# matsengrp/linearham

Hardware: AMD Instinct MI355X
Metric: phylo-HMM log-likelihood evals/sec (100-leaf x 400-site family) (higher is better)
Workload: dtype f64

## Files before the change

### include/linearham_amd.h

```cpp
#ifndef LINEARHAM_AMD_H_
#define LINEARHAM_AMD_H_

#include <stddef.h>
#include <stdint.h>

#ifdef __cplusplus
extern "C" {
#endif

#define LH_ABI_VERSION 1

typedef struct lh_family lh_family;

typedef struct {
  int32_t n_genes;
  const int32_t* offsets;
  const int32_t* xmsa_inds;
} lh_segments;

typedef struct {
  int32_t n_rows;
  int32_t n_left;
  int32_t n_right;
  const double* enter_trans;
// ... 31 lines not shown
} lh_family_desc;

typedef struct {
  double* rates;
  double* xmsa_emission;
  double* forward;
  int32_t* scaler_counts;
} lh_eval_outputs;

const char* lh_last_error(void);
int lh_device_count(void);

int lh_warmup(void);
int lh_set_device(int32_t device);
void* lh_host_alloc(size_t bytes);
void lh_host_free(void* p);

int lh_family_create(const lh_family_desc* desc, lh_family** out);
void lh_family_destroy(lh_family* fam);

int64_t lh_forward_size(const lh_family* fam);
int64_t lh_scaler_size(const lh_family* fam);

int lh_family_info(const lh_family* fam, int32_t* n_patterns, int32_t* n_unique_columns);

int lh_family_consensus_sets(const lh_family* fam);

const char* lh_family_prune_form(const lh_family* fam);

const char* lh_family_forward_form(const lh_family* fam);

int lh_family_forward_dj_samples(const lh_family* fam);

int lh_family_set_extended_range(lh_family* fam, int enable);

typedef struct {
  int32_t n_rows, n_left, n_right, n_states;
  const int32_t* left_rows;
  const int32_t* left_dense;
  const double* left_lo;
  const double* left_trans;
  const double* enter_lo;
  const int32_t* right_dense;
  const int32_t* right_first;
  const double* gene_prob;
  const double* nti_landing_in;
  const double* nti_transition;
  const double* nti_landing_out;
  const double* landing_in;
  const double* right_trans;
  const double* exit_nlo;
  const double* exit_trans;
  const double* exit_li;
  const double* prod;
} lh_sampler_junction;

typedef struct {
  lh_sampler_junction vd, dj;
} lh_sampler_desc;

int lh_family_set_sampler(lh_family* fam, const lh_sampler_desc* desc);

int32_t lh_sample_words(const lh_family* fam);
int32_t lh_sample_states(const lh_family* fam);

int lh_eval_sample_batch(lh_family* fam, int32_t n, int32_t n_tips, int32_t max_depth, const int32_t* ops,
// ... 317 lines not shown
```

### linearham_amd/capi.py

```python
import ctypes as C
import os

import numpy as np

_HERE = os.path.dirname(os.path.abspath(__file__))

c_i32p = C.POINTER(C.c_int32)
c_u8p = C.POINTER(C.c_uint8)
c_f64p = C.POINTER(C.c_double)


class _Segments(C.Structure):
    _fields_ = [("n_genes", C.c_int32), ("offsets", c_i32p), ("xmsa_inds", c_i32p)]


class _Junction(C.Structure):
    _fields_ = [("n_rows", C.c_int32), ("n_left", C.c_int32), ("n_right", C.c_int32),
                ("enter_trans", c_f64p), ("enter_lo", c_f64p), ("left_trans", c_f64p),
                ("left_lo", c_f64p), ("left_xmsa", c_i32p), ("right_gp_nli", c_f64p),
                ("right_ntt", c_f64p), ("right_nlo", c_f64p), ("right_trans", c_f64p),
                ("right_gp_li", c_f64p), ("right_xmsa", c_i32p), ("nti_xmsa", c_i32p),
                ("exit_nlo", c_f64p), ("exit_trans", c_f64p), ("exit_gp_li", c_f64p)]


class _FamilyDesc(C.Structure):
    _fields_ = [("abi_version", C.c_int32), ("has_d", C.c_int32), ("n_seqs", C.c_int32),
                ("n_sites", C.c_int32), ("msa", c_u8p), ("n_xmsa", C.c_int32),
                ("xmsa_site", c_i32p), ("xmsa_naive_base", c_u8p),
                ("vpadding", _Segments), ("vgerm", _Segments), ("dgerm", _Segments),
                ("jgerm", _Segments), ("jpadding", _Segments),
                ("vgerm_gene_prob", c_f64p), ("vpadding_transition", c_f64p),
                ("vgerm_trans_prod", c_f64p), ("jpadding_transition", c_f64p),
                ("vd", _Junction), ("dj", _Junction)]


class _EvalOutputs(C.Structure):
    _fields_ = [("rates", c_f64p), ("xmsa_emission", c_f64p), ("forward", c_f64p),
                ("scaler_counts", c_i32p)]


EXPORTS = ["lh_last_error", "lh_device_count", "lh_family_create", "lh_family_destroy",
           "lh_forward_size", "lh_scaler_size", "lh_family_info", "lh_family_consensus_sets", "lh_schedule_tree", "lh_eval_batch",
           "lh_eval_batch_device", "lh_forward_batch", "lh_asr_batch", "lh_asr_batch_device",
           "lh_profile_enable", "lh_profile_read", "lh_asr_profile_read", "lh_family_set_extended_range", "lh_warmup", "lh_host_alloc", "lh_host_free", "lh_family_set_sampler",
           "lh_sample_words", "lh_sample_states", "lh_eval_sample_batch", "lh_set_device", "lh_family_status",
           "lh_eval_sample_batch_device", "lh_family_prune_form", "lh_family_forward_form",
           "lh_family_forward_dj_samples"]
POSTERIOR_EXPORTS = ["lh_eval_posterior_batch", "lh_eval_posterior_batch_device", "lh_posterior_profile_read"]
EXPORTS += POSTERIOR_EXPORTS
CANDIDATE_EXPORTS = ["lh_family_set_candidates", "lh_eval_candidates_batch", "lh_eval_candidates_batch_device",
                     "lh_candidates_profile_read", "lh_candidates_info", "lh_candidates_layout"]
EXPORTS += CANDIDATE_EXPORTS
COLLECT_EXPORTS = ["lh_eval_draw_batch", "lh_eval_draw_batch_device", "lh_naive_sequences", "lh_draws_resolve",
                   "lh_draws_rows_read", "lh_draws_candidates_read", "lh_draws_reset", "lh_collect_profile_read"]
EXPORTS += COLLECT_EXPORTS
LINEAGE_EXPORTS = ["lh_lineage_batch", "lh_lineage_collect_device", "lh_lineage_resolve", "lh_lineage_rows_read",
                   "lh_lineage_store_read", "lh_lineage_reset", "lh_lineage_profile_read"]
EXPORTS += LINEAGE_EXPORTS
LINEAGE_PAD_HASH = 0
LINEAGE_EVAL_EXPORTS = ["lh_eval_lineage_batch", "lh_eval_lineage_batch_device", "lh_lineage_eval_profile_read"]
EXPORTS += LINEAGE_EVAL_EXPORTS
VITERBI_EXPORTS = ["lh_eval_viterbi_batch", "lh_eval_viterbi_batch_device", "lh_viterbi_forward_batch",
                   "lh_family_set_candidate_paths", "lh_viterbi_profile_read"]
EXPORTS += VITERBI_EXPORTS
CODON_EXPORTS = ["lh_family_set_codons", "lh_codon_layout", "lh_eval_codons_batch", "lh_eval_codons_batch_device",
                 "lh_codon_profile_read"]
EXPORTS += CODON_EXPORTS
EVENTS_EXPORTS = ["lh_events_layout", "lh_eval_events_batch", "lh_eval_events_batch_device", "lh_events_forward_batch",
                  "lh_events_profile_read"]
EXPORTS += EVENTS_EXPORTS
ANCESTRAL_EXPORTS = ["lh_asr_marginals_batch", "lh_asr_marginals_batch_device", "lh_eval_ancestral_batch",
                     "lh_eval_ancestral_batch_device", "lh_ancestral_profile_read"]
EXPORTS += ANCESTRAL_EXPORTS
EDGES_EXPORTS = ["lh_asr_edges_batch", "lh_asr_edges_batch_device", "lh_eval_edges_batch", "lh_eval_edges_batch_device",
                 "lh_edges_profile_read"]
EXPORTS += EDGES_EXPORTS
ANCESTRAL_PROBS_EXPORTS = ["lh_family_set_ancestral_candidates", "lh_ancestral_candidates_info",
                           "lh_eval_ancestral_candidates_batch", "lh_eval_ancestral_candidates_batch_device",
                           "lh_ancestral_candidates_profile_read"]
EXPORTS += ANCESTRAL_PROBS_EXPORTS
# ... 113 lines not shown
_HOST_TREE = [C.c_void_p, C.c_int32, C.c_int32, C.c_int32, c_i32p, c_f64p, c_f64p, c_f64p, c_f64p, C.c_int32]
_DEV_TREE = [C.c_void_p, C.c_int32, C.c_int32, C.c_int32] + [C.c_void_p] * 5 + [C.c_int32]
_PROFILE_READ = [C.c_void_p, c_f64p, C.POINTER(C.c_int64)]


class HipLibrary:
    def __init__(self, path=None):
        path = path or library_path()
        if not os.path.exists(path):
            raise RuntimeError("HIP library %s is missing: run `python -c 'import __graft_entry__ as g; "
                               "g.build()'` (there is no CPU fallback)" % path)
        self.lib = lib = C.CDLL(path)
        c_u32p, c_u64p = C.POINTER(C.c_uint32), C.POINTER(C.c_uint64)
        lib.lh_last_error.restype = C.c_char_p
        lib.lh_device_count.restype = C.c_int
        lib.lh_family_create.argtypes = [C.POINTER(_FamilyDesc), C.POINTER(C.c_void_p)]
        lib.lh_family_destroy.argtypes = [C.c_void_p]
        lib.lh_family_destroy.restype = None
        lib.lh_forward_size.argtypes = [C.c_void_p]
        lib.lh_forward_size.restype = C.c_int64
        lib.lh_scaler_size.argtypes = [C.c_void_p]
        lib.lh_scaler_size.restype = C.c_int64
        lib.lh_family_info.argtypes = [C.c_void_p, C.POINTER(C.c_int32), C.POINTER(C.c_int32)]
        lib.lh_family_info.restype = C.c_int
        lib.lh_family_consensus_sets.argtypes = [C.c_void_p]
        lib.lh_family_consensus_sets.restype = C.c_int
        lib.lh_family_prune_form.argtypes = [C.c_void_p]
        lib.lh_family_prune_form.restype = C.c_char_p
        lib.lh_family_forward_form.argtypes = [C.c_void_p]
        lib.lh_family_forward_form.restype = C.c_char_p
        if hasattr(lib, "lh_family_forward_dj_samples"):
            lib.lh_family_forward_dj_samples.argtypes = [C.c_void_p]
            lib.lh_family_forward_dj_samples.restype = C.c_int
        lib.lh_schedule_tree.argtypes = [C.c_int32, c_i32p, C.c_int32, c_i32p, c_i32p]
        lib.lh_eval_batch.argtypes = _HOST_TREE + [c_f64p, C.POINTER(_EvalOutputs)]
        lib.lh_eval_batch_device.argtypes = _DEV_TREE + [C.c_void_p, C.POINTER(_EvalOutputs), C.c_void_p]
        lib.lh_forward_batch.argtypes = [C.c_void_p, C.c_int32, c_f64p, c_f64p, C.POINTER(_EvalOutputs)]
        lib.lh_asr_batch.argtypes = _HOST_TREE + [c_u8p, C.c_uint64, C.c_uint64, c_u8p, c_u8p]
        lib.lh_asr_batch_device.argtypes = _DEV_TREE + [C.c_void_p, C.c_uint64, C.c_uint64] + [C.c_void_p] * 3
        lib.lh_asr_profile_read.argtypes = _PROFILE_READ
        lib.lh_profile_enable.argtypes = [C.c_void_p, C.c_int]
        lib.lh_family_set_extended_range.argtypes = [C.c_void_p, C.c_int]
        lib.lh_profile_read.argtypes = [C.c_void_p, c_f64p, c_f64p, c_f64p, C.POINTER(C.c_int64)]
        if hasattr(lib, "lh_eval_sample_batch_device"):
            lib.lh_eval_sample_batch_device.argtypes = _DEV_TREE + [C.c_void_p] * 5
            lib.lh_sample_words.argtypes = [C.c_void_p]
            lib.lh_sample_states.argtypes = [C.c_void_p]
        if hasattr(lib, "lh_eval_posterior_batch"):
            lib.lh_eval_posterior_batch.argtypes = _HOST_TREE + [C.POINTER(_PosteriorOutputs)]
            lib.lh_eval_posterior_batch_device.argtypes = _DEV_TREE + [C.POINTER(_PosteriorOutputs), C.c_void_p]
            lib.lh_posterior_profile_read.argtypes = _PROFILE_READ
        if hasattr(lib, "lh_family_set_candidates"):
            lib.lh_family_set_candidates.argtypes = [C.c_void_p, C.c_int32, c_u8p, c_f64p]
            lib.lh_eval_candidates_batch.argtypes = _HOST_TREE + [C.POINTER(_CandidateOutputs)]
            lib.lh_eval_candidates_batch_device.argtypes = _DEV_TREE + [C.POINTER(_CandidateOutputs), C.c_void_p]
            lib.lh_candidates_profile_read.argtypes = _PROFILE_READ
            lib.lh_candidates_info.argtypes = [C.c_void_p, c_i32p, c_i32p]
            lib.lh_candidates_layout.argtypes = [C.c_void_p, c_i32p, c_i32p, c_i32p]
        if hasattr(lib, "lh_naive_sequences"):
            lib.lh_eval_draw_batch.argtypes = _HOST_TREE + [c_u32p, c_f64p, c_u64p, c_i32p]
            lib.lh_eval_draw_batch_device.argtypes = _DEV_TREE + [C.c_void_p] * 5
            lib.lh_naive_sequences.argtypes = [C.c_void_p, C.c_int32, c_i32p, c_u8p, c_u64p]
            lib.lh_draws_resolve.argtypes = [C.c_void_p, C.c_int32, c_i32p, c_i32p, c_i32p]
            lib.lh_draws_rows_read.argtypes = [C.c_void_p, C.c_int32, c_i32p, c_u8p]
            lib.lh_draws_candidates_read.argtypes = [C.c_void_p, c_i32p, c_u8p]
            lib.lh_draws_reset.argtypes = [C.c_void_p]
# ... 618 lines not shown

    def eval_batch(self, n_tips, max_depth, ops, brlen, er, pi, alpha, num_rates, want=()):
        _, arrays = _tree_args(ops, brlen, er, pi, alpha)
        ops, brlen, er, pi, alpha = arrays
        n = alpha.shape[0]
        assert ops.shape == (n, n_tips - 2, 4) and brlen.shape == (n, 2 * n_tips - 2)
        assert er.shape == (n, 6) and pi.shape == (n, 4)
        ll = np.zeros(n)
        outs, res = self._outs(n, num_rates, want)
        self.hip.check(self.hip.lib.lh_eval_batch(self.handle, n, n_tips, max_depth, *_tree_ptrs(arrays), num_rates,
                                                  _ptr(ll), C.byref(outs)))
        return ll, res

    def eval_batch_device(self, n, n_tips, max_depth, ops_ptr, brlen_ptr, er_ptr, pi_ptr, alpha_ptr,
                          num_rates, loglik_ptr, stream=0):
        self.hip.check(self.hip.lib.lh_eval_batch_device(
            self.handle, n, n_tips, max_depth, ops_ptr, brlen_ptr, er_ptr, pi_ptr, alpha_ptr, num_rates,
            loglik_ptr, None, stream))

    def info(self):
        a, b = C.c_int32(), C.c_int32()
        self.hip.check(self.hip.lib.lh_family_info(self.handle, C.byref(a), C.byref(b)))
        return a.value, b.value

    def k1_form(self):
        return self.hip.lib.lh_family_prune_form(self.handle).decode()

    def k2_form(self):
        return self.hip.lib.lh_family_forward_form(self.handle).decode()

    def k2_dj_samples(self):
        return int(self.hip.lib.lh_family_forward_dj_samples(self.handle))

    def status(self):
        self.hip.check(self.hip.lib.lh_family_status(self.handle))

    def forward_batch(self, em, want=()):
        em = _f64(em)
        n = em.shape[0]
        assert em.shape == (n, self.n_xmsa)
        ll = np.zeros(n)
        outs, res = self._outs(n, 1, [w for w in want if w in ("forward", "scaler_counts")])
        self.hip.check(self.hip.lib.lh_forward_batch(self.handle, n, em.ctypes.data_as(c_f64p),
                                                     ll.ctypes.data_as(c_f64p), C.byref(outs)))
        return ll, res

    def asr_batch(self, n_tips, max_depth, ops, brlen, er, pi, rates, naive, seed, first_sample=0):
        _, arrays = _tree_args(ops, brlen, er, pi, rates)
        ops, brlen, er, pi, rates = arrays
        naive = np.ascontiguousarray(naive, dtype=np.uint8)
        n, L = naive.shape
        assert ops.shape == (n, n_tips - 2, 4) and brlen.shape == (n, 2 * n_tips - 2)
        assert er.shape == (n, 6) and pi.shape == (n, 4) and rates.shape[0] == n
        anc = np.zeros((n, n_tips - 2, L), dtype=np.uint8)
        choice = np.zeros((n, L), dtype=np.uint8)
        self.hip.check(self.hip.lib.lh_asr_batch(self.handle, n, n_tips, max_depth, *_tree_ptrs(arrays), rates.shape[1],
                                                 _ptr(naive, c_u8p), seed, first_sample, _ptr(anc, c_u8p),
                                                 _ptr(choice, c_u8p)))
        return anc, choice

    def asr_marginals_batch(self, n_tips, max_depth, ops, brlen, er, pi, rates, naive_prob, path,
                            want=("marg", "rate_post")):
        _, arrays = _tree_args(ops, brlen, er, pi, rates)
        ops, brlen, er, pi, rates = arrays
        naive_prob = _f64(naive_prob)
        path = _i32(path)
# ... 161 lines not shown
```

### linearham_amd/csrc/lh_capi.hip

```cpp
#include <algorithm>
#include <array>
#include <map>
#include <cstdio>
#include <cstring>
#include <functional>
#include <atomic>
#include <chrono>
#include <string>
#include <thread>
#include <utility>
#include <vector>

#include "lh_device.h"

namespace lh {
const DebugOptions& debug_options() {
  static const DebugOptions opts = [] {
    DebugOptions o;
    auto set = [](const char* name) { return std::getenv(name) != nullptr; };
    auto num = [](const char* name, int dflt) { const char* e = std::getenv(name); return e ? std::atoi(e) : dflt; };
    o.chunk = std::max(256, num("LH_CHUNK", o.chunk));
    o.host_sub = std::max(256, num("LH_HOST_SUB", o.host_sub));
    o.eval_split = std::min(8, std::max(0, num("LH_EVAL_SPLIT", o.eval_split)));
    o.k0_serial = set("LH_K0_SERIAL");
    o.eval_fwd_priority = std::min(1, num("LH_EVAL_FWD_PRIORITY", o.eval_fwd_priority));
    o.k2b_no_pair = set("LH_K2B_NO_PAIR");
    o.k2b_vd_single = set("LH_K2B_VD_SINGLE");
    o.k2b_dj_pair = set("LH_K2B_DJ_PAIR");
    o.sample_timing = set("LH_SAMPLE_TIMING");
    o.k1_tile_cap = num("LH_K1_TILE_CAP", 0);
    o.k1_cxx_walk = set("LH_K1_CXX_WALK");
    o.k1_tables = set("LH_K1_TABLES");
    o.k1_stack = set("LH_K1_STACK");
    o.k1_no_tables = set("LH_K1_NO_TABLES");
    o.k1_segments = set("LH_K1_SEGMENTS");
    o.k1_seg_waves = num("LH_K1_SEG_WAVES", o.k1_seg_waves);
    o.k1_no_fuse = set("LH_K1_NO_FUSE");
    o.codon_blocks = std::max(1, num("LH_CODON_BLOCKS", o.codon_blocks));
    o.events_blocks = std::max(1, num("LH_EVENTS_BLOCKS", o.events_blocks));
    o.anc_out_mb = std::max(1, num("LH_ANC_OUT_MB", o.anc_out_mb));
    o.edge_out_mb = std::max(1, num("LH_EDGE_OUT_MB", o.edge_out_mb));
    o.anc_pairs = std::max(0, num("LH_ANC_PAIRS", o.anc_pairs));
    o.collect_hash_bits = std::min(64, std::max(1, num("LH_COLLECT_HASH_BITS", o.collect_hash_bits)));
    return o;
  }();
  return opts;
}
}

namespace {

thread_local std::string g_error;

int fail(const std::string& msg) {
  g_error = msg;
  return 1;
}

#define LH_HIP(expr)                                                                      \
  do {                                                                                    \
// ... 539 lines not shown
  std::vector<T> t(rows * n_pad * inner, fill);
  for (size_t i = 0; i < rows; ++i)
    for (size_t g = 0; g < n; ++g)
      for (size_t u = 0; u < inner; ++u) t[(i * n_pad + g) * inner + u] = src[(i * n + g) * inner + u];
  return t;
}

template <typename T>
int upload_vec(lh_family* f, const std::vector<T>& v, const T** out) {
  return upload(f, v.data(), v.size(), out);
}

int upload_junction(lh_family* f, const lh_junction& j, const std::vector<int32_t>& remap, int n_jcols,
                    const int32_t* xmsa_site, const std::vector<int32_t>& pat_of_site, int left_chunks, int right_chunks,
                    lh::DevJunction* d) {
  const size_t W = j.n_rows, nL = j.n_left, nR = j.n_right;
  const size_t pL = std::max<size_t>((nL + 63) / 64, (size_t)left_chunks) * 64,
               pR = std::max<size_t>((nR + 63) / 64, (size_t)right_chunks) * 64;
  d->n_rows = j.n_rows;
  d->n_left = j.n_left;
  d->n_right = j.n_right;
  d->left_pad = (int32_t)pL;
  d->right_pad = (int32_t)pR;
  if (!j.enter_trans || !j.enter_lo || !j.left_trans || !j.left_lo || !j.right_gp_nli || !j.right_ntt ||
      !j.right_nlo || !j.right_trans || !j.right_gp_li || !j.exit_nlo || !j.exit_trans || !j.exit_gp_li)
    return fail("lh_family_create: null array in junction descriptor");
  auto cols = [&](const int32_t* src, size_t rows, size_t n, size_t n_pad, size_t inner) {
    std::vector<int32_t> t = pad_genes<int32_t>(src, rows, n, n_pad, inner, -1);
    for (int32_t& x : t) x = x >= 0 ? remap[x] : n_jcols;
    return t;
  };
  std::vector<double> ltr = pad_genes<double>(j.left_trans, W, nL, pL, 1, 0.0);
  for (size_t l = 0; l < nL; ++l) ltr[l] = j.enter_trans[l];
  std::vector<double> ntt(pR * 16, 0.0);
  for (size_t r = 0; r < nR; ++r)
    for (int a = 0; a < 4; ++a)
      for (int b = 0; b < 4; ++b) ntt[r * 16 + b * 4 + a] = j.right_ntt[r * 16 + a * 4 + b];
  if (upload_vec(f, pad_genes<double>(j.enter_lo, 1, nL, pL, 1, 0.0), &d->enter_lo)) return 1;
  if (upload_vec(f, ltr, &d->left_trans)) return 1;
  if (upload_vec(f, pad_genes<double>(j.left_lo, W, nL, pL, 1, 0.0), &d->left_lo)) return 1;
  if (upload_vec(f, cols(j.left_xmsa, W, nL, pL, 1), &d->left_xmsa)) return 1;
  if (upload_vec(f, pad_genes<double>(j.right_gp_nli, 1, nR, pR, 4, 0.0), &d->right_gp_nli)) return 1;
  if (upload_vec(f, ntt, &d->right_ntt)) return 1;
  if (upload_vec(f, pad_genes<double>(j.right_nlo, W, nR, pR, 4, 0.0), &d->right_nlo)) return 1;
  if (upload_vec(f, pad_genes<double>(j.right_trans, W, nR, pR, 1, 0.0), &d->right_trans)) return 1;
  if (upload_vec(f, pad_genes<double>(j.right_gp_li, W, nR, pR, 1, 0.0), &d->right_gp_li)) return 1;
  if (upload_vec(f, cols(j.right_xmsa, W, nR, pR, 1), &d->right_xmsa)) return 1;
  if (upload_vec(f, cols(j.nti_xmsa, W, nR, pR, 4), &d->nti_xmsa)) return 1;
  if (upload_vec(f, pad_genes<double>(j.exit_nlo, 1, nR, pR, 4, 0.0), &d->exit_nlo)) return 1;
  if (upload_vec(f, pad_genes<double>(j.exit_trans, 1, nR, pR, 1, 0.0), &d->exit_trans)) return 1;
  if (upload_vec(f, pad_genes<double>(j.exit_gp_li, 1, nR, pR, 1, 0.0), &d->exit_gp_li)) return 1;
  std::vector<int32_t> row_pat(W, f->host.n_prune);
  if (xmsa_site)
    for (size_t i = 0; i < W; ++i) row_pat[i] = pat_of_site[xmsa_site[j.nti_xmsa[i * nR * 4]]];
  if (upload_vec(f, row_pat, &d->row_pat)) return 1;
  return 0;
}

size_t k1_bytes_per_sample(const lh_family* f, int T, int R) {
  const lh::PruneWsSizes z = lh::prune_ws_sizes(T, f->host.msa_mixed_n != 0);
  const size_t n_ops = (size_t)std::max(T - 2, 1);
  return sizeof(double) * R * z.scratch_doubles_per_rate + n_ops * (sizeof(int2) + sizeof(double)) +
         z.tabs_per_sample * sizeof(int4) + sizeof(int4);
}

int ensure_workspace(lh_family* f, int n, int R, int T) {
// ... 563 lines not shown
  if (!rc && desc->n_seqs > 0) {
    rc = upload(f, desc->xmsa_site, C, &f->cand.col_site) || upload(f, desc->xmsa_naive_base, C, &f->cand.col_base);
    lh_family_desc d2 = *desc;
    d2.n_seqs = 0;
    d2.msa = nullptr;
    const std::string keep = g_error;
    if (!rc && lh_family_create(&d2, &f->cand.twin)) f->cand.twin_error = g_error;
    g_error = keep;
  }
  if (rc) {
    std::string keep = g_error;
    lh_family_destroy(f);
    g_error = keep;
    return 1;
  }
  *out = f;
  return 0;
}

void lh_family_destroy(lh_family* f) {
  if (!f) return;
  DeviceGuard guard(f);
  lh_family_destroy(std::exchange(f->cand.twin, nullptr));
  for (void* p : f->allocs) (void)hipFree(p);
  delete f;
}

int64_t lh_forward_size(const lh_family* f) { return f ? f->host.forward_size : 0; }

const char* lh_family_prune_form(const lh_family* f) { return f ? f->k1_form.c_str() : ""; }

const char* lh_family_forward_form(const lh_family* f) { return f ? f->k2_form.c_str() : ""; }
int lh_family_forward_dj_samples(const lh_family* f) { return f ? f->k2_dj_samples : 0; }

int lh_family_consensus_sets(const lh_family* f) {
  if (!f) return 0;
  const lh::DevFamily& h = f->host;
  return (h.vpadding.cons_sites > 0) | (h.vgerm.cons_sites > 0) << 1 | (h.dgerm.cons_sites > 0) << 2 |
         (h.jgerm.cons_sites > 0) << 3 | (h.jpadding.cons_sites > 0) << 4;
}

int lh_family_info(const lh_family* f, int32_t* n_patterns, int32_t* n_unique_columns) {
  if (!f) return fail("lh_family_info: null family");
  if (n_patterns) *n_patterns = f->host.n_prune;
  if (n_unique_columns) *n_unique_columns = f->n_ucol_used;
  return 0;
}
int64_t lh_scaler_size(const lh_family* f) { return f ? f->host.scaler_size : 0; }

int lh_schedule_tree(int32_t T, const int32_t* children, int32_t root, int32_t* ops, int32_t* max_depth) {
  if (T < 3) return fail("lh_schedule_tree: need at least 3 tips (naive + 2 sequences)");
  const int n_nodes = 2 * T - 2, I = T - 2;
  if (!children || !ops) return fail("lh_schedule_tree: null argument");
  if (root < T || root >= n_nodes) return fail("lh_schedule_tree: root must be an inner node");
  std::vector<int> seen(n_nodes, 0);
  for (int i = 0; i < 2 * I; ++i) {
    const int c = children[i];
    if (c < 1 || c >= n_nodes) return fail("lh_schedule_tree: child id out of range");
    if (seen[c]++) return fail("lh_schedule_tree: node appears twice as a child");
  }
  if (seen[root]) return fail("lh_schedule_tree: root appears as a child");
  for (int v = 1; v < n_nodes; ++v)
    if (v != root && !seen[v]) return fail("lh_schedule_tree: node is not attached to the tree");
  std::vector<int> size(n_nodes, 0), order;
  order.reserve(I);
  {
// ... 2615 lines not shown
```

### linearham_amd/csrc/lh_device.h

```cpp
#pragma once
#include <hip/hip_runtime.h>
#include <stdint.h>

#include <functional>

#include "linearham_amd.h"

namespace lh {

constexpr double kScaleFactor = 0x1p256;
constexpr double kScaleThreshold = 0x1p-256;
constexpr double kLogScaleFactor = 177.445678223345993274;

template <class... P, class... A>
static inline void launch_lds(void (*kernel)(P...), dim3 grid, dim3 block, size_t lds, hipStream_t stream,
                              const A&... args) {
  if (lds > 64 * 1024)
    (void)hipFuncSetAttribute(reinterpret_cast<const void*>(kernel), hipFuncAttributeMaxDynamicSharedMemorySize, (int)lds);
  hipLaunchKernelGGL(kernel, grid, block, lds, stream, args...);
}

enum : int { OP_CHERRY = 0, OP_TIP_ACC = 1, OP_POP_ACC = 2, OP_PUSH_FLAG = 16, OP_RANK_SHIFT = 8 };

enum : int { W_CHERRY = 0, W_TIP_ACC = 1, W_POP = 2, W_CTIP = 3, W_CTAB_ACC = 4 };

struct PruneWs {
  double* scratch;
  int2* wops;
  double* wlen;
  int4* tabs;
  int4* hdr;
  int32_t* err_flag;
};
struct PruneWsSizes {
  size_t scratch_doubles_per_rate;
  size_t tabs_per_sample;
};
PruneWsSizes prune_ws_sizes(int T, bool mixed_n);
struct PruneFork {
  hipStream_t sched;
  std::function<int()> join;
};

struct DevSegments {
  int32_t n_genes;
  int32_t n_chunks;
  int32_t cons_sites;
  int32_t cons_diffs;
  const uint16_t* cons_col;
  const uint32_t* cons_rng;
  const uint32_t* cons_dif;
  const uint4* inds_c;
};

struct DevJunction {
  int32_t n_rows, n_left, n_right;
  int32_t left_pad, right_pad;
  const double *enter_lo;
  const double *left_trans;
  const double *left_lo;
  const int32_t* left_xmsa;
  const double *right_gp_nli;
  const double *right_ntt;
  const double *right_nlo;
  const double *right_trans, *right_gp_li;
  const int32_t *right_xmsa;
  const int32_t *nti_xmsa;
  const double *exit_nlo;
  const double *exit_trans, *exit_gp_li;
  const int32_t* row_pat;
};

struct DevFamily {
  int32_t has_d, n_seqs, n_sites, n_xmsa;
  int32_t n_pat;
  int32_t n_prune;
  int32_t msa_mixed_n;
  int32_t n_ucol;
  int32_t idx_byte_offsets;
  const uint8_t* msa;
  const uint64_t* msa_planes;
  const int32_t* site_pat;
  const int32_t* u_pat;
  const uint8_t* u_base;
  const int32_t* ucol_of_col;
  const int32_t* col_of_ucol;
  DevSegments vpadding, vgerm, dgerm, jgerm, jpadding;
  const double *vgerm_gene_prob, *vpadding_transition, *vgerm_trans_prod, *jpadding_transition;
  DevJunction vd, dj;
  int32_t max_genes;
// ... 364 lines not shown
void launch_pair_finish(int K, long long q0, int count, const double* pair_ll, const double* open_ll, const int32_t* plen,
                        double* log_cand, double* prob, hipStream_t stream);

struct LogEmRequest {
  const int32_t* cols = nullptr;
  int n = 0;
  double* out = nullptr;
};
void launch_forward(const DevFamily& fam, const DevFamily* fam_dev, int n, int R, const double* site_lik,
                    const int32_t* site_scal, const double* pi, const double* em_in, double* em_out, double* gem,
                    int32_t* gcnt, double* jem,
                    int32_t* jrs, double* dxf, int32_t* dxc, double* loglik, double* forward_out, int32_t* scaler_out,
                    bool extended, hipStream_t stream, const LogEmRequest& lem = LogEmRequest{});
size_t forward_lds_bytes(const DevFamily& fam);
const char* forward_last_form();
int forward_last_dj_samples();

size_t viterbi_bp_bytes(const DevFamily& fam);
size_t viterbi_lds_bytes(const DevFamily& fam);
void launch_viterbi(const DevFamily& fam, const DevSampler* smp_dev, int n, const double* gem, const int32_t* gcnt,
                    const double* jem, const int32_t* jrs, const double* loglik, uint8_t* bp, int32_t* states,
                    double* log_path, bool extended, hipStream_t stream);
void launch_path_prior(const DevFamily& fam, const DevSampler* smp_dev, int K, const int32_t* states, double* log_prior,
                       int32_t* first_bad, hipStream_t stream);

struct DebugOptions {
  int chunk = 49152;
  int host_sub = 12288;
  int eval_split = 0;
  bool k0_serial = false;
  int eval_fwd_priority = -1;
  bool k2b_no_pair = false;
  bool k2b_vd_single = false;
  bool k2b_dj_pair = false;
  bool sample_timing = false;
  int k1_tile_cap = 0;
  bool k1_cxx_walk = false;
  bool k1_tables = false;
  bool k1_stack = false;
  bool k1_no_tables = false;
  bool k1_segments = false;
  int k1_seg_waves = 4;
  bool k1_no_fuse = false;
  int codon_blocks = 2048;
  int events_blocks = 1024;
  int anc_out_mb = 4096;
  int edge_out_mb = 4096;
  int anc_pairs = 0;
  int collect_hash_bits = 64;
};
const DebugOptions& debug_options();

}
```

### linearham_amd/csrc/lh_forward.hip

```cpp
#include <cstdio>
#include <cstdlib>
#include <type_traits>

#include "lh_device.h"

namespace lh {

constexpr int kFwdThreads = 256;
constexpr int kFwdWaves = kFwdThreads / 64;
constexpr int kJunctionWaves = 4;

thread_local char g_k2a_form[64] = "", g_k2b_form[32] = "", g_forward_form[160] = "";
thread_local int g_k2b_dj_samples = 0;

__device__ static inline int block_max_int(int v, int* red, int phase) {
#pragma unroll
  for (int off = 32; off > 0; off >>= 1) v = max(v, __shfl_xor(v, off, 64));
  int* r = red + phase * kFwdWaves;
  if ((threadIdx.x & 63) == 0) r[threadIdx.x >> 6] = v;
  __syncthreads();
  return max(max(r[0], r[1]), max(r[2], r[3]));
}

__device__ static inline int block_min_int(int v, int* red, int phase) {
// ... 583 lines not shown
}

template <bool kExt>
__device__ static inline unsigned key_start() {
  return kExt ? 0u : 0xffffffffu;
}
template <bool kExt>
__device__ static inline unsigned key_add(unsigned key, double v) {
  return kExt ? max(key, (unsigned)__double2hiint(v)) : min(key, scale_key(v));
}

struct RowScale {
  int k;
  double factor;
  bool extra;
  __device__ double apply(double v) const {
    v *= factor;
    if (extra) v *= kScaleFactor;
    return v;
  }
};

__device__ static inline RowScale row_scale(unsigned min_key) {
  const unsigned hw = min_key + 1u;
  const unsigned e = (hw >> 20) & 0x7ffu;
  RowScale s;
  s.extra = hw != 0 && e == 0 && (hw & 0xfffffu) < (1u << 18);
  const int k3 = hw == 0 ? 0 : (e < 767u) + (e < 511u) + (e < 255u);
  s.k = k3 + (s.extra ? 1 : 0);
  s.factor = __hiloint2double((1023 + 256 * k3) << 20, 0);
  return s;
}

template <bool kExt>
__device__ static inline RowScale wave_row_scale(unsigned key) {
  return row_scale(kExt ? wave_max_u32(key) - 1u : wave_min_key(key));
}

__device__ static __forceinline__ RowScale pick(bool hi, const RowScale& sa, const RowScale& sb) {
  return RowScale{hi ? sb.k : sa.k, hi ? sb.factor : sa.factor, hi ? sb.extra : sa.extra};
}

struct RightRow {
  double nlo[4], rtr, rli;
  int ridx;
  int4 nx;
};

template <int GL, int GR>
struct RowTables {
  double ltr[GL], llo[GL];
  int lidx[GL];
  RightRow right[GR];
};

__device__ static __forceinline__ void load_right_row(const DevJunction& J, int i, unsigned r, RightRow& t) {
  const size_t orr = (size_t)i * J.right_pad;
  const double2* pn = reinterpret_cast<const double2*>(J.right_nlo) + 2 * orr;
  const double2 a = pn[2u * r], b = pn[2u * r + 1u];
  t.nlo[0] = a.x;
  t.nlo[1] = a.y;
  t.nlo[2] = b.x;
  t.nlo[3] = b.y;
  t.nx = (reinterpret_cast<const int4*>(J.nti_xmsa) + orr)[r];
  t.rtr = (J.right_trans + orr)[r];
  t.rli = (J.right_gp_li + orr)[r];
// ... 227 lines not shown
      const double v = (fL * ltr) * jem[lidx];
      fL = v;
      key = key_add<kExt>(key, v);
    }
    const double part = fL * llo;
    key = right_gene_step<kExt>(key, fN, fR, A, nli, ntt_lds, g, t, jem);
    A = mine(half_sums(part));
    const HalfKeys hk = half_keys<kExt>(key);
    const RowScale sa = row_scale(hk.a), sb = row_scale(hk.b);
    if constexpr (kExt) count += jrs[i];
    if ((sa.k | sb.k) != 0) {
      const RowScale sc = pick(hi, sa, sb);
      A = sc.apply(A);
      fL = sc.apply(fL);
      fR = sc.apply(fR);
#pragma unroll
      for (int b = 0; b < 4; ++b) fN[b] = sc.apply(fN[b]);
      count += sc.k;
    }
    if (fwd_out && valid) {
      double* o = fwd_out + (size_t)i * row_stride;
      if ((int)g < nL) o[g] = fL;
      store_right(o, nL, nR, g, fN, fR);
    }
    if (scal_out && valid && g == 0) scal_out[i] = count;
  }
  g_out = exit_handoff(J, g, nR, fN, fR, A, germ_em, pad_trans, pad_em);
  const HalfKeys hk = half_keys<kExt>(key_add<kExt>(key_start<kExt>(), g_out));
  const RowScale last = pick(hi, row_scale(hk.a), row_scale(hk.b));
  g_out = last.apply(g_out);
  return count + last.k;
}

template <int GL, bool kExt>
__device__ static void junction_vd_pair(const DevJunction& J, const double* jemA, const double* jemB,
                                        const double* ntt_lds, int lane, bool hi, const double (&fA_in)[GL],
                                        const double (&fB_in)[GL], int countA_in, int countB_in,
                                        const double* __restrict__ germ_em_mine, double& g_out, int& count_mine,
                                        double* __restrict__ fwdA, double* __restrict__ fwdB,
                                        int32_t* __restrict__ scoA, int32_t* __restrict__ scoB,
                                        const int32_t* __restrict__ jrsA, const int32_t* __restrict__ jrsB) {
  const int W = J.n_rows, nL = J.n_left, nR = J.n_right;
  const unsigned g = lane & 31;
  const double* jemM = hi ? jemB : jemA;
  int countA = countA_in, countB = countB_in;
  double fA[GL], fB[GL], fN[4] = {0.0, 0.0, 0.0, 0.0}, fR = 0.0, nli[4];
#pragma unroll
  for (int q = 0; q < GL; ++q) {
    fA[q] = fA_in[q];
    fB[q] = fB_in[q];
  }
  load_nli(J, g, nli);
  const size_t row_stride = (size_t)nL + 5 * (size_t)nR;
  double AA, AB;
  {
    double pa = 0.0, pb = 0.0;
#pragma unroll
    for (int q = 0; q < GL; ++q) {
      const double lo = J.enter_lo[lane + 64u * q];
      pa += fA_in[q] * lo;
      pb += fB_in[q] * lo;
    }
    AA = wave_sum(pa);
    AB = wave_sum(pb);
  }
  auto combine = [](unsigned a, unsigned b) { return kExt ? max(a, b) : min(a, b); };
  for (int i = 0; i < W; ++i) {
    const size_t ol = (size_t)i * J.left_pad;
    unsigned keyA = key_start<kExt>(), keyB = key_start<kExt>();
    double partA = 0.0, partB = 0.0;
    {
      const double* lt = J.left_trans + ol;
      const double* ll = J.left_lo + ol;
      const int32_t* lx = J.left_xmsa + ol;
#pragma unroll
      for (int q = 0; q < GL; ++q) {
        const double ltr = lt[lane + 64u * q], llo = ll[lane + 64u * q];
        const int lidx = lx[lane + 64u * q];
        const double va = (fA[q] * ltr) * jemA[lidx];
        const double vb = (fB[q] * ltr) * jemB[lidx];
        fA[q] = va;
        fB[q] = vb;
        keyA = key_add<kExt>(keyA, va);
        keyB = key_add<kExt>(keyB, vb);
        partA += va * llo;
        partB += vb * llo;
      }
    }
    {
      RightRow t;
      load_right_row(J, i, g, t);
      const unsigned keyR = right_gene_step<kExt>(key_start<kExt>(), fN, fR, hi ? AB : AA, nli, ntt_lds, g, t, jemM);
      if (hi)
        keyB = combine(keyB, keyR);
      else
        keyA = combine(keyA, keyR);
    }
    AA = wave_sum(partA);
    AB = wave_sum(partB);
    const RowScale sa = wave_row_scale<kExt>(keyA), sb = wave_row_scale<kExt>(keyB);
    if constexpr (kExt) {
      countA += jrsA[i];
      countB += jrsB[i];
    }
    if ((sa.k | sb.k) != 0) {
      AA = sa.apply(AA);
      AB = sb.apply(AB);
#pragma unroll
      for (int q = 0; q < GL; ++q) {
        fA[q] = sa.apply(fA[q]);
        fB[q] = sb.apply(fB[q]);
      }
      const RowScale sm = pick(hi, sa, sb);
      fR = sm.apply(fR);
#pragma unroll
      for (int b = 0; b < 4; ++b) fN[b] = sm.apply(fN[b]);
      countA += sa.k;
      countB += sb.k;
    }
    if (fwdA) {
      double* oa = fwdA + (size_t)i * row_stride;
      double* ob = fwdB ? fwdB + (size_t)i * row_stride : nullptr;
#pragma unroll
      for (int q = 0; q < GL; ++q) {
        const int t = lane + 64 * q;
        if (t < nL) {
          oa[t] = fA[q];
          if (ob) ob[t] = fB[q];
        }
      }
      double* om = hi ? ob : oa;
      if (om) store_right(om, nL, nR, g, fN, fR);
    }
    if (lane == 0) {
      if (scoA) scoA[i] = countA;
      if (scoB) scoB[i] = countB;
    }
  }
// ... 62 lines not shown
                       const int32_t* __restrict__ gcnt_all, const double* __restrict__ jem_all,
                       const int32_t* __restrict__ jrs_all, double* __restrict__ fwd_all,
                       int32_t* __restrict__ scal_all, double* __restrict__ dxf, int32_t* __restrict__ dxc) {
  extern __shared__ double jlds[];
  const int lane = threadIdx.x & 63, wave = threadIdx.x >> 6;
  const int s = blockIdx.x * kJunctionWaves + wave;
  const int NJ = fam.n_jcols;
  double* ntt_vd = jlds;
  double* jem = ntt_vd + 16 * (size_t)fam.vd.right_pad + (size_t)wave * (NJ + 1);
  stage_ntt(ntt_vd, fam.vd.right_ntt, 16 * fam.vd.right_pad, 64 * kJunctionWaves);
  __syncthreads();
  if (s >= n) return;
  const int nV = fam.vgerm.n_genes, nD = fam.dgerm.n_genes;
  const size_t vd_fwd = junction_fwd_size(fam.vd);
  stage_jem<1>(jem, jem_all, s, n, NJ, lane);
  const double* gem = gem_all + (size_t)s * fam.gem_size;
  const int cv = gcnt_all[(size_t)s * 3 + 0], cd = gcnt_all[(size_t)s * 3 + 1];
  double* fwd = fwd_all ? fwd_all + (size_t)s * fam.forward_size : nullptr;
  int32_t* sco = scal_all ? scal_all + (size_t)s * fam.scaler_size : nullptr;
  double gV[GA];
  const int vcount = initial_v_forward<GA, kExt>(fam, gem, lane, cv, gV, fwd, sco);
  double gD[1];
  const int dcount =
      cd + junction_wave<GA, 1, kExt>(fam.vd, jem, ntt_vd, lane, gV, vcount, gem + 2 * (size_t)nV, nullptr, nullptr, gD,
                                      fwd ? fwd + nV : nullptr, sco ? sco + 1 : nullptr,
                                      kExt ? jrs_all + (size_t)s * (fam.vd.n_rows + fam.dj.n_rows) : nullptr);
  if (fwd && lane < nD) fwd[nV + vd_fwd + lane] = gD[0];
  if (sco && lane == 0) sco[1 + fam.vd.n_rows] = dcount;
  if (lane < 32) dxf[(size_t)s * 32 + lane] = gD[0];
  if (lane == 0) dxc[s] = dcount;
}

constexpr int kVdPairWaves = 4;
template <int GA, bool kExt>
__global__ void __launch_bounds__(64 * kVdPairWaves)
    junction_vd2_kernel(const DevFamily fam, int n, const double* __restrict__ gem_all,
                        const int32_t* __restrict__ gcnt_all, const double* __restrict__ jem_all,
                        const int32_t* __restrict__ jrs_all, double* __restrict__ fwd_all,
                        int32_t* __restrict__ scal_all, double* __restrict__ dxf, int32_t* __restrict__ dxc) {
  extern __shared__ double jlds[];
  const int lane = threadIdx.x & 63, wave = threadIdx.x >> 6;
  const int NJ = fam.n_jcols;
  double* ntt_vd = jlds;
  double* jem0 = ntt_vd + 16 * (size_t)fam.vd.right_pad + (size_t)(2 * wave) * (NJ + 1);
  stage_ntt(ntt_vd, fam.vd.right_ntt, 16 * fam.vd.right_pad, 64 * kVdPairWaves);
  __syncthreads();
  const int p = blockIdx.x * kVdPairWaves + wave;
  if (2 * p >= n) return;
  const bool hi = lane >= 32;
  const int sA = 2 * p, sB = min(2 * p + 1, n - 1);
  const bool validB = 2 * p + 1 < n;
  stage_jem<2>(jem0, jem_all, sA, n, NJ, lane);
  const int nV = fam.vgerm.n_genes, nD = fam.dgerm.n_genes;
  const size_t vd_fwd = junction_fwd_size(fam.vd);
  const double* gemA = gem_all + (size_t)sA * fam.gem_size;
  const double* gemB = gem_all + (size_t)sB * fam.gem_size;
  double* fwdA = fwd_all ? fwd_all + (size_t)sA * fam.forward_size : nullptr;
  double* fwdB = fwd_all && validB ? fwd_all + (size_t)sB * fam.forward_size : nullptr;
  int32_t* scoA = scal_all ? scal_all + (size_t)sA * fam.scaler_size : nullptr;
  int32_t* scoB = scal_all && validB ? scal_all + (size_t)sB * fam.scaler_size : nullptr;
  double gA[GA], gB[GA];
  unsigned keyA = key_start<kExt>(), keyB = key_start<kExt>();
#pragma unroll
  for (int q = 0; q < GA; ++q) {
    const int t = lane + 64 * q;
    double va = 0.0, vb = 0.0;
    if (t < nV) {
// ... 10 lines not shown
      vb *= gemB[nV + t];
    }
    keyA = key_add<kExt>(keyA, va);
    keyB = key_add<kExt>(keyB, vb);
    gA[q] = va;
    gB[q] = vb;
  }
  int countA = gcnt_all[(size_t)sA * 3 + 0], countB = gcnt_all[(size_t)sB * 3 + 0];
  {
    const RowScale sa = wave_row_scale<kExt>(keyA), sb = wave_row_scale<kExt>(keyB);
#pragma unroll
    for (int q = 0; q < GA; ++q) {
      gA[q] = sa.apply(gA[q]);
      gB[q] = sb.apply(gB[q]);
    }
    countA += sa.k;
    countB += sb.k;
  }
  if (fwdA) {
#pragma unroll
    for (int q = 0; q < GA; ++q)
      if (lane + 64 * q < nV) {
        fwdA[lane + 64 * q] = gA[q];
        if (fwdB) fwdB[lane + 64 * q] = gB[q];
      }
  }
  if (lane == 0) {
    if (scoA) scoA[0] = countA;
    if (scoB) scoB[0] = countB;
  }
  const size_t jr = (size_t)fam.vd.n_rows + fam.dj.n_rows;
  double gD;
  int count_mine;
  junction_vd_pair<GA, kExt>(fam.vd, jem0, jem0 + (NJ + 1), ntt_vd, lane, hi, gA, gB, countA, countB,
                             (hi ? gemB : gemA) + 2 * (size_t)nV, gD, count_mine, fwdA ? fwdA + nV : nullptr,
                             fwdB ? fwdB + nV : nullptr, scoA ? scoA + 1 : nullptr, scoB ? scoB + 1 : nullptr,
                             kExt ? jrs_all + (size_t)sA * jr : nullptr, kExt ? jrs_all + (size_t)sB * jr : nullptr);
  const unsigned g = lane & 31;
  const int dcount = gcnt_all[(size_t)(hi ? sB : sA) * 3 + 1] + count_mine;
  if (!hi || validB) {
    const int sM = hi ? sB : sA;
    double* fwdM = hi ? fwdB : fwdA;
    int32_t* scoM = hi ? scoB : scoA;
    if (fwdM && (int)g < nD) fwdM[nV + vd_fwd + g] = gD;
    if (scoM && g == 0) scoM[1 + fam.vd.n_rows] = dcount;
    dxf[(size_t)sM * 32 + g] = gD;
    if (g == 0) dxc[sM] = dcount;
  }
}

constexpr int kPairWaves = 4;

struct DjSample {
  const double *jgerm_em, *jpad_em;
  int cj;
  double* fwd;
  int32_t* sco;
  const int32_t* jrs;
};

template <bool kExt>
__device__ static __forceinline__ DjSample dj_sample(const DevFamily& fam, int s, const double* __restrict__ gem_all,
                                                     const int32_t* __restrict__ gcnt_all,
                                                     const int32_t* __restrict__ jrs_all, double* __restrict__ fwd_all,
                                                     int32_t* __restrict__ scal_all) {
  const int nV = fam.vgerm.n_genes, nD = fam.dgerm.n_genes, nJ = fam.jgerm.n_genes;
  DjSample d;
  d.jgerm_em = gem_all + (size_t)s * fam.gem_size + 2 * (size_t)nV + nD;
  d.jpad_em = d.jgerm_em + nJ;
  d.cj = gcnt_all[(size_t)s * 3 + 2];
// ... 362 lines not shown

template <bool kExt>
static void launch_dj(const DevFamily& fam, int n, const double* gem, const int32_t* gcnt, const double* jem,
                      const int32_t* jrs, const double* dxf, const int32_t* dxc, double* loglik, double* forward_out,
                      int32_t* scaler_out, hipStream_t stream) {
  const size_t lds_dj = ((size_t)2 * kPairWaves * (fam.n_jcols + 1) + 16 * (size_t)fam.dj.right_pad) * sizeof(double);
  const int waves = dj4_waves(fam, lds_dj);
  g_k2b_dj_samples = waves == 0 ? 2 : 4;
  auto kernel = junction_dj_kernel<kExt>;
  size_t lds = lds_dj;
  dim3 grid(((n + 1) / 2 + kPairWaves - 1) / kPairWaves), block(64 * kPairWaves);
  if (waves != 0) {
    kernel = fam.dgerm.n_genes <= 16 ? junction_dj4_kernel<1, kExt> : junction_dj4_kernel<2, kExt>;
    lds = dj4_lds_bytes(fam, waves);
    grid = dim3(((n + 3) / 4 + waves - 1) / waves);
    block = dim3(64 * waves);
  }
  launch_lds(kernel, grid, block, lds, stream, fam, n, gem, gcnt, jem, jrs, dxf, dxc, loglik, forward_out, scaler_out);
}

template <int GA, int GB>
static void launch_junction_g(const DevFamily& fam, int n, const double* gem, const int32_t* gcnt, const double* jem,
                              const int32_t* jrs, double* dxf, int32_t* dxc, double* loglik, double* forward_out,
                              int32_t* scaler_out, bool ext, hipStream_t stream) {
  g_k2b_dj_samples = 0;
  if constexpr (GB == 1) {
    if (junction_pair_form(fam)) {
      const size_t jem_slice = (size_t)fam.n_jcols + 1, ntt_vd = 16 * (size_t)fam.vd.right_pad;
      bool vd2 = false;
      if constexpr (GA <= 4) {
        static const bool vd_single = debug_options().k2b_vd_single;
        vd2 = !vd_single;
      }
      snprintf(g_k2b_form, sizeof(g_k2b_form), vd2 ? "vd2<%d>+dj" : "vd<%d>+dj", GA);
      with_bool(ext, [&](auto E) {
        constexpr bool kE = decltype(E)::value;
        if constexpr (GA <= 4) {
          if (vd2)
            launch_lds(junction_vd2_kernel<GA, kE>, dim3(((n + 1) / 2 + kVdPairWaves - 1) / kVdPairWaves),
                       dim3(64 * kVdPairWaves), (2 * kVdPairWaves * jem_slice + ntt_vd) * sizeof(double), stream, fam, n,
                       gem, gcnt, jem, jrs, forward_out, scaler_out, dxf, dxc);
        }
        if (!vd2)
          launch_lds(junction_vd_kernel<GA, kE>, dim3((n + kJunctionWaves - 1) / kJunctionWaves),
                     dim3(64 * kJunctionWaves), (kJunctionWaves * jem_slice + ntt_vd) * sizeof(double), stream, fam, n,
                     gem, gcnt, jem, jrs, forward_out, scaler_out, dxf, dxc);
        launch_dj<kE>(fam, n, gem, gcnt, jem, jrs, dxf, dxc, loglik, forward_out, scaler_out, stream);
      });
      return;
    }
  }
  snprintf(g_k2b_form, sizeof(g_k2b_form), "junction<%d,%d>", GA, GB);
  with_bool(ext, [&](auto E) {
    launch_lds(junction_kernel<GA, GB, decltype(E)::value>, dim3((n + kJunctionWaves - 1) / kJunctionWaves),
               dim3(64 * kJunctionWaves), junction_lds_bytes(fam), stream, fam, n, gem, gcnt, jem, jrs, loglik,
               forward_out, scaler_out);
  });
}

template <int GA>
static void launch_junction_a(int gb, const DevFamily& fam, int n, const double* gem, const int32_t* gcnt,
                              const double* jem, const int32_t* jrs, double* dxf, int32_t* dxc, double* loglik,
                              double* forward_out, int32_t* scaler_out, bool ext, hipStream_t stream) {
  if (gb <= 1)
    launch_junction_g<GA, 1>(fam, n, gem, gcnt, jem, jrs, dxf, dxc, loglik, forward_out, scaler_out, ext, stream);
  else if (gb <= 2)
    launch_junction_g<GA, 2>(fam, n, gem, gcnt, jem, jrs, dxf, dxc, loglik, forward_out, scaler_out, ext, stream);
  else
    launch_junction_g<GA, 4>(fam, n, gem, gcnt, jem, jrs, dxf, dxc, loglik, forward_out, scaler_out, ext, stream);
}

void launch_forward(const DevFamily& fam, const DevFamily* fam_dev, int n, int R, const double* site_lik,
                    const int32_t* site_scal, const double* pi, const double* em_in, double* em_out, double* gem,
                    int32_t* gcnt, double* jem, int32_t* jrs, double* dxf, int32_t* dxc, double* loglik,
// ... 40 lines not shown
```

Before: 8.534 million.

## Skip dead VD left rows and merge rescale key reductions in vd2 kernel

At family creation, the host finds trailing VD junction rows whose left transitions are all zero with no emissions and records how many live left rows there are. In the paired VD kernel, once past those rows, a wave ballot checks that no left value is infinite or NaN. If so, the left contributions are zeroed and the per-row left dot products and wave sums are skipped. The scale keys for both samples are also combined with a lane permute into one wave reduction and a cheaper rescale test, and the old path is kept behind an environment flag.

```diff
diff --git a/include/linearham_amd.h b/include/linearham_amd.h
--- a/include/linearham_amd.h
+++ b/include/linearham_amd.h
@@ -87,6 +87,8 @@
 
 int lh_family_forward_dj_samples(const lh_family* fam);
 
+int lh_family_vd_left_rows(const lh_family* fam);
+
 int lh_family_set_extended_range(lh_family* fam, int enable);
 
 typedef struct {
diff --git a/linearham_amd/capi.py b/linearham_amd/capi.py
--- a/linearham_amd/capi.py
+++ b/linearham_amd/capi.py
@@ -45,7 +45,7 @@
            "lh_profile_enable", "lh_profile_read", "lh_asr_profile_read", "lh_family_set_extended_range", "lh_warmup", "lh_host_alloc", "lh_host_free", "lh_family_set_sampler",
            "lh_sample_words", "lh_sample_states", "lh_eval_sample_batch", "lh_set_device", "lh_family_status",
            "lh_eval_sample_batch_device", "lh_family_prune_form", "lh_family_forward_form",
-           "lh_family_forward_dj_samples"]
+           "lh_family_forward_dj_samples", "lh_family_vd_left_rows"]
 POSTERIOR_EXPORTS = ["lh_eval_posterior_batch", "lh_eval_posterior_batch_device", "lh_posterior_profile_read"]
 EXPORTS += POSTERIOR_EXPORTS
 CANDIDATE_EXPORTS = ["lh_family_set_candidates", "lh_eval_candidates_batch", "lh_eval_candidates_batch_device",
@@ -225,6 +225,9 @@
         if hasattr(lib, "lh_family_forward_dj_samples"):
             lib.lh_family_forward_dj_samples.argtypes = [C.c_void_p]
             lib.lh_family_forward_dj_samples.restype = C.c_int
+        if hasattr(lib, "lh_family_vd_left_rows"):
+            lib.lh_family_vd_left_rows.argtypes = [C.c_void_p]
+            lib.lh_family_vd_left_rows.restype = C.c_int
         lib.lh_schedule_tree.argtypes = [C.c_int32, c_i32p, C.c_int32, c_i32p, c_i32p]
         lib.lh_eval_batch.argtypes = _HOST_TREE + [c_f64p, C.POINTER(_EvalOutputs)]
         lib.lh_eval_batch_device.argtypes = _DEV_TREE + [C.c_void_p, C.POINTER(_EvalOutputs), C.c_void_p]
@@ -909,6 +912,9 @@
     def k2_dj_samples(self):
         return int(self.hip.lib.lh_family_forward_dj_samples(self.handle))
 
+    def vd_left_rows(self):
+        return int(self.hip.lib.lh_family_vd_left_rows(self.handle))
+
     def status(self):
         self.hip.check(self.hip.lib.lh_family_status(self.handle))
 
diff --git a/linearham_amd/csrc/lh_capi.hip b/linearham_amd/csrc/lh_capi.hip
--- a/linearham_amd/csrc/lh_capi.hip
+++ b/linearham_amd/csrc/lh_capi.hip
@@ -6,6 +6,7 @@
 #include <functional>
 #include <atomic>
 #include <chrono>
+#include <cmath>
 #include <string>
 #include <thread>
 #include <utility>
@@ -26,6 +27,7 @@
     o.eval_fwd_priority = std::min(1, num("LH_EVAL_FWD_PRIORITY", o.eval_fwd_priority));
     o.k2b_no_pair = set("LH_K2B_NO_PAIR");
     o.k2b_vd_single = set("LH_K2B_VD_SINGLE");
+    o.k2b_vd_plain = set("LH_K2B_VD_PLAIN");
     o.k2b_dj_pair = set("LH_K2B_DJ_PAIR");
     o.sample_timing = set("LH_SAMPLE_TIMING");
     o.k1_tile_cap = num("LH_K1_TILE_CAP", 0);
@@ -631,6 +633,16 @@
   };
   std::vector<double> ltr = pad_genes<double>(j.left_trans, W, nL, pL, 1, 0.0);
   for (size_t l = 0; l < nL; ++l) ltr[l] = j.enter_trans[l];
+  size_t left_rows = W;
+  auto dead_row = [&](size_t i) {
+    for (size_t l = 0; l < nL; ++l) {
+      const double t = ltr[i * pL + l];
+      if (t != 0.0 || std::signbit(t) || j.left_xmsa[i * nL + l] >= 0 || !std::isfinite(j.left_lo[i * nL + l])) return false;
+    }
+    return true;
+  };
+  while (left_rows > 0 && dead_row(left_rows - 1)) --left_rows;
+  d->left_rows = (int32_t)left_rows;
   std::vector<double> ntt(pR * 16, 0.0);
   for (size_t r = 0; r < nR; ++r)
     for (int a = 0; a < 4; ++a)
@@ -1260,6 +1272,7 @@
 
 const char* lh_family_forward_form(const lh_family* f) { return f ? f->k2_form.c_str() : ""; }
 int lh_family_forward_dj_samples(const lh_family* f) { return f ? f->k2_dj_samples : 0; }
+int lh_family_vd_left_rows(const lh_family* f) { return f ? f->host.vd.left_rows : 0; }
 
 int lh_family_consensus_sets(const lh_family* f) {
   if (!f) return 0;
diff --git a/linearham_amd/csrc/lh_device.h b/linearham_amd/csrc/lh_device.h
--- a/linearham_amd/csrc/lh_device.h
+++ b/linearham_amd/csrc/lh_device.h
@@ -56,6 +56,7 @@
 struct DevJunction {
   int32_t n_rows, n_left, n_right;
   int32_t left_pad, right_pad;
+  int32_t left_rows;
   const double *enter_lo;
   const double *left_trans;
   const double *left_lo;
@@ -486,6 +487,7 @@
   int eval_fwd_priority = -1;
   bool k2b_no_pair = false;
   bool k2b_vd_single = false;
+  bool k2b_vd_plain = false;
   bool k2b_dj_pair = false;
   bool sample_timing = false;
   int k1_tile_cap = 0;
diff --git a/linearham_amd/csrc/lh_forward.hip b/linearham_amd/csrc/lh_forward.hip
--- a/linearham_amd/csrc/lh_forward.hip
+++ b/linearham_amd/csrc/lh_forward.hip
@@ -639,6 +639,11 @@
   return s;
 }
 
+__device__ static inline bool key_rescales(unsigned min_key) {
+  const unsigned hw = min_key + 1u;
+  return hw != 0u && (hw & 0x7fffffffu) < (767u << 20);
+}
+
 template <bool kExt>
 __device__ static inline RowScale wave_row_scale(unsigned key) {
   return row_scale(kExt ? wave_max_u32(key) - 1u : wave_min_key(key));
@@ -932,7 +937,7 @@
   return count + last.k;
 }
 
-template <int GL, bool kExt>
+template <int GL, bool kExt, bool kPlain>
 __device__ static void junction_vd_pair(const DevJunction& J, const double* jemA, const double* jemB,
                                         const double* ntt_lds, int lane, bool hi, const double (&fA_in)[GL],
                                         const double (&fB_in)[GL], int countA_in, int countB_in,
@@ -965,11 +970,27 @@
     AB = wave_sum(pb);
   }
   auto combine = [](unsigned a, unsigned b) { return kExt ? max(a, b) : min(a, b); };
+  bool lean = false;
   for (int i = 0; i < W; ++i) {
-    const size_t ol = (size_t)i * J.left_pad;
+    if (!kPlain && i == J.left_rows) {
+      unsigned top = 0u;
+#pragma unroll
+      for (int q = 0; q < GL; ++q)
+        top = max(top, max((unsigned)__double2hiint(fA[q]), (unsigned)__double2hiint(fB[q])));
+      lean = __builtin_amdgcn_ballot_w64(top >= 0x7ff00000u) == 0;
+      if (lean) {
+#pragma unroll
+        for (int q = 0; q < GL; ++q) fA[q] = fB[q] = 0.0;
+      }
+    }
+    RightRow t;
+    load_right_row(J, i, g, t);
     unsigned keyA = key_start<kExt>(), keyB = key_start<kExt>();
-    double partA = 0.0, partB = 0.0;
-    {
+    unsigned keyL = key_start<kExt>();
+    double nextA = 0.0, nextB = 0.0;
+    if (!lean) {
+      const size_t ol = (size_t)i * J.left_pad;
+      double partA = 0.0, partB = 0.0;
       const double* lt = J.left_trans + ol;
       const double* ll = J.left_lo + ol;
       const int32_t* lx = J.left_xmsa + ol;
@@ -986,24 +1007,40 @@
         partA += va * llo;
         partB += vb * llo;
       }
-    }
-    {
-      RightRow t;
-      load_right_row(J, i, g, t);
-      const unsigned keyR = right_gene_step<kExt>(key_start<kExt>(), fN, fR, hi ? AB : AA, nli, ntt_lds, g, t, jemM);
+      if constexpr (!kPlain) {
+        const auto x = __builtin_amdgcn_permlane32_swap(keyA, keyB, false, false);
+        keyL = combine(x[0], x[1]);
+      }
+      nextA = wave_sum(partA);
+      nextB = wave_sum(partB);
+    }
+    const unsigned keyR = right_gene_step<kExt>(key_start<kExt>(), fN, fR, hi ? AB : AA, nli, ntt_lds, g, t, jemM);
+    AA = nextA;
+    AB = nextB;
+    RowScale sa, sb;
+    HalfKeys hk;
+    bool rescale;
+    if constexpr (kPlain) {
       if (hi)
         keyB = combine(keyB, keyR);
       else
         keyA = combine(keyA, keyR);
-    }
-    AA = wave_sum(partA);
-    AB = wave_sum(partB);
-    const RowScale sa = wave_row_scale<kExt>(keyA), sb = wave_row_scale<kExt>(keyB);
+      sa = wave_row_scale<kExt>(keyA);
+      sb = wave_row_scale<kExt>(keyB);
+      rescale = (sa.k | sb.k) != 0;
+    } else {
+      hk = half_keys<kExt>(combine(keyL, keyR));
+      rescale = key_rescales(hk.a) || key_rescales(hk.b);
+    }
     if constexpr (kExt) {
       countA += jrsA[i];
       countB += jrsB[i];
     }
-    if ((sa.k | sb.k) != 0) {
+    if (rescale) {
+      if constexpr (!kPlain) {
+        sa = row_scale(hk.a);
+        sb = row_scale(hk.b);
+      }
       AA = sa.apply(AA);
       AB = sb.apply(AB);
 #pragma unroll
@@ -1132,7 +1169,7 @@
 }
 
 constexpr int kVdPairWaves = 4;
-template <int GA, bool kExt>
+template <int GA, bool kExt, bool kPlain = false>
 __global__ void __launch_bounds__(64 * kVdPairWaves)
     junction_vd2_kernel(const DevFamily fam, int n, const double* __restrict__ gem_all,
                         const int32_t* __restrict__ gcnt_all, const double* __restrict__ jem_all,
@@ -1209,10 +1246,11 @@
   const size_t jr = (size_t)fam.vd.n_rows + fam.dj.n_rows;
   double gD;
   int count_mine;
-  junction_vd_pair<GA, kExt>(fam.vd, jem0, jem0 + (NJ + 1), ntt_vd, lane, hi, gA, gB, countA, countB,
-                             (hi ? gemB : gemA) + 2 * (size_t)nV, gD, count_mine, fwdA ? fwdA + nV : nullptr,
-                             fwdB ? fwdB + nV : nullptr, scoA ? scoA + 1 : nullptr, scoB ? scoB + 1 : nullptr,
-                             kExt ? jrs_all + (size_t)sA * jr : nullptr, kExt ? jrs_all + (size_t)sB * jr : nullptr);
+  junction_vd_pair<GA, kExt, kPlain>(fam.vd, jem0, jem0 + (NJ + 1), ntt_vd, lane, hi, gA, gB, countA, countB,
+                                     (hi ? gemB : gemA) + 2 * (size_t)nV, gD, count_mine, fwdA ? fwdA + nV : nullptr,
+                                     fwdB ? fwdB + nV : nullptr, scoA ? scoA + 1 : nullptr, scoB ? scoB + 1 : nullptr,
+                                     kExt ? jrs_all + (size_t)sA * jr : nullptr,
+                                     kExt ? jrs_all + (size_t)sB * jr : nullptr);
   const unsigned g = lane & 31;
   const int dcount = gcnt_all[(size_t)(hi ? sB : sA) * 3 + 1] + count_mine;
   if (!hi || validB) {
@@ -1641,14 +1679,16 @@
         static const bool vd_single = debug_options().k2b_vd_single;
         vd2 = !vd_single;
       }
-      snprintf(g_k2b_form, sizeof(g_k2b_form), vd2 ? "vd2<%d>+dj" : "vd<%d>+dj", GA);
+      static const bool vd_plain = debug_options().k2b_vd_plain;
+      snprintf(g_k2b_form, sizeof(g_k2b_form), !vd2 ? "vd<%d>+dj" : vd_plain ? "vd2plain<%d>+dj" : "vd2<%d>+dj", GA);
       with_bool(ext, [&](auto E) {
         constexpr bool kE = decltype(E)::value;
         if constexpr (GA <= 4) {
           if (vd2)
-            launch_lds(junction_vd2_kernel<GA, kE>, dim3(((n + 1) / 2 + kVdPairWaves - 1) / kVdPairWaves),
-                       dim3(64 * kVdPairWaves), (2 * kVdPairWaves * jem_slice + ntt_vd) * sizeof(double), stream, fam, n,
-                       gem, gcnt, jem, jrs, forward_out, scaler_out, dxf, dxc);
+            launch_lds(vd_plain ? junction_vd2_kernel<GA, kE, true> : junction_vd2_kernel<GA, kE, false>,
+                       dim3(((n + 1) / 2 + kVdPairWaves - 1) / kVdPairWaves), dim3(64 * kVdPairWaves),
+                       (2 * kVdPairWaves * jem_slice + ntt_vd) * sizeof(double), stream, fam, n, gem, gcnt, jem, jrs,
+                       forward_out, scaler_out, dxf, dxc);
         }
         if (!vd2)
           launch_lds(junction_vd_kernel<GA, kE>, dim3((n + kJunctionWaves - 1) / kJunctionWaves),
```

New measurement: 8.617 million (median of 6 runs). No clear change (+1.0%).
